# zhongyuanzhao/dl_ofdm

Measured on AMD Instinct MI355X. Metric: OFDM symbols/sec fwd+bwd, DCCN QPSK N=64, higher is better.
Workload: dtype f32; 1 GPU; QPSK, N=64/CP=16, batch=8192 OFDM symbols (1170 frames x 7), fwd+bwd+Adam; nfft=64, cp=16, nfilter=64, nbits=2, parallelism=independent batch per GPU, final all-reduce of the BER/loss table

## Files before the change

dl_ofdm_amd/csrc/dccn_abi.hip:

```cpp
#include "abi_impl.h"

namespace dccn {
thread_local int g_last_hip_error = 0;
thread_local ChainCtx tl_chain = {1, {{0, 0, 0, 0, 0, 0, 0, 0}}, {0, 0, 0, 0, 0, 0, 0, 0}, {0, 0, 0, 0, 0, 0, 0, 0}, {0, 0, 0, 0, 0, 0, 0, 0}, {0, 0, 0, 0, 0, 0, 0, 0}};
StepTraceState g_step_trace;
thread_local unsigned long long* tl_stamp = nullptr;

thread_local int tl_whole_k = -1;
thread_local int tl_tune_depth = 0;
thread_local int tl_tune_vals[TUNE_COUNT];
TuneTable g_tune = {{{9}, {7}, {7}, {7}, {0}, {0}, {0}, {1}, {1}, {1}, {1}, {1}, {3}, {1}, {14}, {0}, {0}, {1}, {0}, {2}, {1}, {1}, {0}, {0}, {1}, {2}, {0}, {1}}};
std::atomic<int> g_whole_k_global{1};

static int norm_grid_x(int cols) { return ceil_div(ceil_div(cols, 4), 64); }
static int norm_grid_y(int batch) { return ceil_div(batch, kNormRowsPerBlock); }

int norm_fused_blocks(int cols) { return ceil_div(ceil_div(cols, 4 * kNormFusedCG), 8) * 8; }
struct NormWs {
    double *moments, *power;
    size_t slots;
    double* power_slot(int slot) const { return power + (slot ? slots : 0); }
};
static NormWs norm_carve(Carver& c, int batch, int cols) {
    const size_t a = (size_t)norm_grid_x(cols) * norm_grid_y(batch), b = (size_t)norm_fused_blocks(cols), slots = a > b ? a : b;
// ... 651 lines not shown
    if (2 * kin == 160) DCCN_TRY(launch_rx_bwd_fused<5>(px, pw, de, nsplit, nr, fin, hp, s));
    else DCCN_TRY(launch_rx_bwd_fused<4>(px, pw, de, nsplit, nr, fin, hp, s));
    *ds = deferred_slabs(sw, dbias_dense != nullptr, true);
    fd->slabs = cw.partial; fd->colsum = cw.colsum;
    fd->splits = ceil_div(batch, 64) * S;
    fd->slab = (long long)((2 * F) / 64) * kin * 64;
    *fold_tilew = 64;
    return DCCN_OK;
}

static int tail_blocks(long long cells, bool quad4 = false) {
    long long b = ceil_div_ll(quad4 ? 4 * cells : cells, kTailThreads);
    const long long cap = quad4 ? kTailBlocksMax : kTailBlocks;
    if (b > cap) b = cap;
    if (b < 1) b = 1;
    return (int)b;
}
struct TailWs { TailBlockMetrics* blk_metrics; float* blk_grads; };
static TailWs tail_carve(Carver& c, size_t nblocks, int nbits) {
    TailBlockMetrics* bm = c.take<TailBlockMetrics>(nblocks);
    return TailWs{bm, c.take<float>(nblocks * tail_param_count(nbits))};
}
size_t tail_ws_bytes(long long cells, int nbits) {
    (void)cells;
    return carved_bytes([&](Carver& c) { tail_carve(c, kTailBlocksMax, nbits); });
}
static TailFinalizeArgs tail_finalize_args(const TailWs& w, int nblocks, bool bwd, int nbits, long long cells, dccn_metrics* metrics,
                                           float* dtailp, const PowerPartials* pp, float* power_out) {
    const bool pw = pp != nullptr && power_out != nullptr;
    TailFinalizeArgs fa{};
    fa.blk_metrics = w.blk_metrics; fa.blk_grads = bwd ? w.blk_grads : nullptr; fa.nblocks = nblocks;
    fa.P = bwd ? tail_param_count(nbits) : 0; fa.count = cells * nbits;
    fa.metrics = metrics; fa.dtailp = bwd ? dtailp : nullptr; fa.power_partial = pw ? pp->partial : nullptr;
    fa.n_power = pw ? pp->n : 0; fa.power_denom = pw ? pp->denom : 1.0; fa.power_out = pw ? power_out : nullptr;
    return fa;
}
static int tail_finish(const TailFinalizeArgs& fa, TailFinalizeArgs* defer, hipStream_t s) {
    if (defer) {
        *defer = fa;
        return DCCN_OK;
    }
    hipLaunchKernelGGL(demod_tail_finalize_kernel, dim3(tail_finalize_blocks(fa.P)), dim3(256), 0, s, fa);
    DCCN_LAUNCH_CHECK();
    return DCCN_OK;
}

template <int NB>
static int tail_launch(bool bwd, const float* z, const int32_t* bits, const float* tailp, float* prob, float* dz,
                       long long cells, int nblk, TailBlockMetrics* bm, float* bg, hipStream_t s) {
    if (bwd)
        DCCN_LAUNCH_CHAINS_Z((demod_tail_kernel<NB, true>), dim3(nblk), dim3(kTailThreads), 0, s, z, bits, tailp, prob,
                             dz, cells, bm, bg);
    else
        DCCN_LAUNCH_CHAINS_Z((demod_tail_kernel<NB, false>), dim3(nblk), dim3(kTailThreads), 0, s, z, bits, tailp, prob,
                             dz, cells, bm, bg);
    DCCN_LAUNCH_CHECK();
    return DCCN_OK;
}

int tail_impl(bool bwd, const float* z, const int32_t* bits, const float* tailp, float* prob,
                     dccn_metrics* metrics, float* dz, float* dtailp, long long cells, int nbits,
                     const PowerPartials* pp, float* power_out, void* ws, size_t ws_bytes, hipStream_t s,
                     TailFinalizeArgs* defer) {
    if (!z || !bits || !tailp || !metrics || cells <= 0 || nbits < 1 || nbits > 4) return DCCN_ERR_INVALID_ARG;
    if (bwd && (!dz || !dtailp)) return DCCN_ERR_INVALID_ARG;
    if (!ws || ws_bytes < tail_ws_bytes(cells, nbits)) return DCCN_ERR_WORKSPACE;
    Carver c(ws, ws_bytes);
    const TailWs tw = tail_carve(c, kTailBlocksMax, nbits);
    TailBlockMetrics* bm = tw.blk_metrics; float* bg = tw.blk_grads;
    const int nblk = tail_blocks(cells, bwd && nbits == 4);
    int st = DCCN_ERR_INVALID_ARG;
    switch (nbits) {
        case 1: st = tail_launch<1>(bwd, z, bits, tailp, prob, dz, cells, nblk, bm, bg, s); break;
        case 2: st = tail_launch<2>(bwd, z, bits, tailp, prob, dz, cells, nblk, bm, bg, s); break;
        case 3: st = tail_launch<3>(bwd, z, bits, tailp, prob, dz, cells, nblk, bm, bg, s); break;
        case 4:
            if (bwd) {
                if (prob)
                    DCCN_LAUNCH_CHAINS_Z(demod_tail_quad4_kernel<true>, dim3(nblk), dim3(kTailThreads), 0, s, z, bits, tailp,
                                         prob, dz, cells, bm, bg, tl_stamp);
                else
                    DCCN_LAUNCH_CHAINS_Z(demod_tail_quad4_kernel<false>, dim3(nblk), dim3(kTailThreads), 0, s, z, bits,
                                         tailp, prob, dz, cells, bm, bg, tl_stamp);
                DCCN_LAUNCH_CHECK();
                st = DCCN_OK;
            } else {
                st = tail_launch<4>(bwd, z, bits, tailp, prob, dz, cells, nblk, bm, bg, s);
            }
            break;
    }
    DCCN_TRY(st);
    if (!defer) DCCN_NO_CHAINS();
    return tail_finish(tail_finalize_args(tw, nblk, bwd, nbits, cells, metrics, dtailp, pp, power_out), defer, s);
}

static int dense_tail_max_blocks(int M, int N) {
    const int b = ceil_div(M, 32) * ceil_div(N, 64);
    const int few = (M <= 96 && (N % 16) == 0) ? ceil_div(M, 16) * (N / 16) : 0;
    return few > b && few <= kTailBlocksMax ? few : b;
}
size_t dense_tail_ws_bytes(int M, int N, int nbits) {
    return carved_bytes([&](Carver& c) { tail_carve(c, (size_t)dense_tail_max_blocks(M, N), nbits); });
}
static bool dense_tail_shape_ok(int M, int K, int N, int nbits) {
    return g_tune[TUNE_DENSE_FWD] > 0 && nbits >= 1 && nbits <= 4 && M > 0 && K > 0 && N > 0 && (K % 4 == 0) && (N % 4 == 0) &&
           small_enough(M, K) && small_enough(K, N) && (long long)ceil_div(M, 128) * ceil_div(N, 128) < 2 * kCUs;
}
bool dense_tail_ok(const float* x, const float* w, int M, int K, int N, int nbits) {
    return dense_tail_shape_ok(M, K, N, nbits) && aligned16(x) && aligned16(w);
}
bool dense_tail_planned(int nbits, bool train, int M, int N) {
    const int k = g_tune[TUNE_TAIL_FUSE_HI];
    if (nbits <= 2) return !((k & 4) && (long long)ceil_div(M, 128) * ceil_div(N, 128) >= 2 * kCUs);
    return (nbits == 4 && train) ? (k & 2) != 0 : (k & 1) != 0;
}

enum DenseGrid : int { DG_TILES = 0, DG_FEWROW, DG_RAGGED };
struct DenseRoute {
    DenseGrid grid;
    bool large;
    int rag;
    int blocks;
};
static DenseRoute dense_tail_route(const GemmParams& p, int nbits) {
    const int M = p.M, N = p.N, ncol = ceil_div(N, 64);
    DenseRoute r{};
    r.large = (long long)ceil_div(M, kDense48.rows()) * ncol >= 4LL * kCUs;
    constexpr int R = kDense80.rows();
    const int rag = (r.large && nbits <= 2 && g_tune[TUNE_DENSE_RAGGED] && M > R) ? M % R : 0;
    const int few_tiles = ceil_div(M, 16) * (N / 16);
    const bool few = g_tune[TUNE_FEWROW] && g_tune[TUNE_SKINNY] > 0 && nbits <= 2 && M <= 96 && fewrow_ng_c(p, false) >= 10 &&
                     few_tiles <= kTailBlocksMax && few_tiles <= dense_tail_max_blocks(M, N);
    if (rag > 0 && rag <= kDense32.rows()) {
        r.grid = DG_RAGGED; r.rag = rag; r.blocks = ((M - rag) / R) * ncol + ncol;
    } else if (few) {
        r.grid = DG_FEWROW; r.blocks = few_tiles;
    } else {
        r.grid = DG_TILES; r.blocks = ceil_div(M, r.large ? R : kDense48.rows()) * ncol;
    }
    return r;
}
static GemmParams split_last_rows(GemmParams& p, int rag) {
    GemmParams q = p;
    p.M -= rag;
    q.M = rag; q.A = p.A + (size_t)p.M * p.lda; q.C = p.C ? p.C + (size_t)p.M * p.ldc : nullptr;
    return q;
}

template <int NB, bool BWD>
static int dense_tail_launch(bool large, const GemmParams& p, const TailEpiParams& tp, hipStream_t s) {
    constexpr Tile16Cfg a = kDense48, b = kDense80;
    const size_t sm = tune_smem_min();
    if (large) return launch_dense_tail16<b.wgm, b.wgn, b.tm, b.tn, b.bk, b.ks, NB, BWD, 2>(p, tp, s, sm);
    return launch_dense_tail16<a.wgm, a.wgn, a.tm, a.tn, a.bk, a.ks, NB, BWD, 2>(p, tp, s, sm);
}

int dense_tail_impl(bool bwd, const float* x, const float* w, const float* bias, float* z, const int32_t* bits,
                           const float* tailp, float* prob, dccn_metrics* metrics, float* dz, float* dtailp, int M,
                           int K, int N, int nbits, const PowerPartials* pp, float* power_out, void* ws, size_t ws_bytes,
                           hipStream_t s, TailFinalizeArgs* defer) {
    if (!x || !w || !bits || !tailp || !metrics || M <= 0 || K <= 0 || N <= 0 || (N & 1) || nbits < 1 || nbits > 4)
        return DCCN_ERR_INVALID_ARG;
    if (bwd && (!dz || !dtailp)) return DCCN_ERR_INVALID_ARG;
    if (!dense_tail_ok(x, w, M, K, N, nbits)) return DCCN_ERR_INVALID_ARG;
    if (!ws || ws_bytes < dense_tail_ws_bytes(M, N, nbits)) return DCCN_ERR_WORKSPACE;
    const GemmParams p = dense_fwd_params(x, w, bias, z, M, K, N);
    if (!vec_both(p)) return DCCN_ERR_INVALID_ARG;
    const DenseRoute r = dense_tail_route(p, nbits);
    Carver c(ws, ws_bytes);
    const TailWs tw = tail_carve(c, (size_t)dense_tail_max_blocks(M, N), nbits);
    const long long cells = (long long)M * (N / 2);
    TailEpiParams tp;
    tp.bits = bits; tp.tailp = tailp; tp.prob = prob; tp.dz = dz; tp.blk_metrics = tw.blk_metrics; tp.blk_grads = tw.blk_grads;
    tp.inv_count = 1.0f / (float)(cells * nbits);
    int st;
    if (r.grid == DG_RAGGED) {
        GemmParams p1 = p;
        const GemmParams p2 = split_last_rows(p1, r.rag);
        const int M1 = p1.M;
        TailEpiParams t2 = tp;
        t2.bits = tp.bits + (size_t)M1 * (N / 2) * nbits;
        t2.prob = tp.prob ? tp.prob + (size_t)M1 * (N / 2) * nbits * 2 : nullptr;
        t2.dz = tp.dz ? tp.dz + (size_t)M1 * N : nullptr;
        constexpr Tile16Cfg c80 = kDense80, c32 = kDense32;
        const size_t sm = tune_smem_min();
        if (nbits == 1) st = bwd ? launch_dense_tail16_ragged<c80.tm, c32.tm, c80.bk, 1, true, 2>(p1, tp, p2, t2, s, sm) : launch_dense_tail16_ragged<c80.tm, c32.tm, c80.bk, 1, false, 2>(p1, tp, p2, t2, s, sm);
        else st = bwd ? launch_dense_tail16_ragged<c80.tm, c32.tm, c80.bk, 2, true, 2>(p1, tp, p2, t2, s, sm) : launch_dense_tail16_ragged<c80.tm, c32.tm, c80.bk, 2, false, 2>(p1, tp, p2, t2, s, sm);
    } else if (r.grid == DG_FEWROW) {
        if (nbits == 1) st = bwd ? launch_fewrow_tail<1, true>(p, tp, s) : launch_fewrow_tail<1, false>(p, tp, s);
        else st = bwd ? launch_fewrow_tail<2, true>(p, tp, s) : launch_fewrow_tail<2, false>(p, tp, s);
    }
    else if (nbits == 1) st = bwd ? dense_tail_launch<1, true>(r.large, p, tp, s) : dense_tail_launch<1, false>(r.large, p, tp, s);
    else if (nbits == 2) st = bwd ? dense_tail_launch<2, true>(r.large, p, tp, s) : dense_tail_launch<2, false>(r.large, p, tp, s);
    else if (nbits == 3) st = bwd ? dense_tail_launch<3, true>(r.large, p, tp, s) : dense_tail_launch<3, false>(r.large, p, tp, s);
    else st = bwd ? dense_tail_launch<4, true>(r.large, p, tp, s) : dense_tail_launch<4, false>(r.large, p, tp, s);
    DCCN_TRY(st);
    return tail_finish(tail_finalize_args(tw, r.blocks, bwd, nbits, cells, metrics, dtailp, pp, power_out), defer, s);
}

static int decide_row_bytes(int D, int nbits) { return (D * nbits + 7) / 8; }
bool decide_outputs_aligned(const float* llr, const float* prob, int nbits) {
    const uintptr_t la = nbits == 4 ? 15u : (nbits == 2 ? 7u : 3u);
    return (reinterpret_cast<uintptr_t>(llr) & la) == 0 && (reinterpret_cast<uintptr_t>(prob) & 7u) == 0;
}

int decide_impl(const float* z, const float* tailp, unsigned char* packed, float* llr, float* prob, int frames, int D,
                int nbits, hipStream_t s) {
    if (!z || !tailp || !packed || frames <= 0 || D <= 0 || nbits < 1 || nbits > 4) return DCCN_ERR_INVALID_ARG;
    if ((reinterpret_cast<uintptr_t>(z) & 7u) != 0 || !decide_outputs_aligned(llr, prob, nbits)) return DCCN_ERR_INVALID_ARG;
    const int gpr = ceil_div(D, 8), RB = decide_row_bytes(D, nbits);
    const long long blocks = ceil_div_ll((long long)frames * gpr * 8, kDecideThreads);
    if (blocks > 0x7fffffffLL) return DCCN_ERR_INVALID_ARG;
    const dim3 grid((unsigned)blocks), blk(kDecideThreads);
    switch (nbits) {
        case 1: DCCN_LAUNCH_CHAINS_Z(demod_decide_kernel<1>, grid, blk, 0, s, z, tailp, packed, llr, prob, frames, D, gpr, RB); break;
        case 2: DCCN_LAUNCH_CHAINS_Z(demod_decide_kernel<2>, grid, blk, 0, s, z, tailp, packed, llr, prob, frames, D, gpr, RB); break;
        case 3: DCCN_LAUNCH_CHAINS_Z(demod_decide_kernel<3>, grid, blk, 0, s, z, tailp, packed, llr, prob, frames, D, gpr, RB); break;
        default: DCCN_LAUNCH_CHAINS_Z(demod_decide_kernel<4>, grid, blk, 0, s, z, tailp, packed, llr, prob, frames, D, gpr, RB); break;
    }
    DCCN_LAUNCH_CHECK();
    return DCCN_OK;
}

int dense_decide_impl(const float* x, const float* w, const float* bias, float* z, const float* tailp, unsigned char* packed,
                      float* llr, float* prob, int M, int K, int N, int nbits, hipStream_t s) {
    if (!x || !w || !tailp || !packed || M <= 0 || K <= 0 || N <= 0 || (N & 1) || nbits < 1 || nbits > 4)
        return DCCN_ERR_INVALID_ARG;
    if (!dense_tail_ok(x, w, M, K, N, nbits)) return DCCN_ERR_INVALID_ARG;
    if (nbits >= 3 && !z) return DCCN_ERR_INVALID_ARG;
    if (!decide_outputs_aligned(llr, prob, nbits)) return DCCN_ERR_INVALID_ARG;
    const GemmParams p = dense_fwd_params(x, w, bias, z, M, K, N);
    if (!vec_both(p)) return DCCN_ERR_INVALID_ARG;
    const size_t sm = tune_smem_min();
    if (nbits >= 3) {
        DCCN_TRY(dense48_launch(p, s, sm));
        return decide_impl(z, tailp, packed, llr, prob, M, N / 2, nbits, s);
    }
    DecideEpiParams dq;
    dq.tailp = tailp; dq.packed = packed; dq.llr = llr; dq.prob = prob; dq.RB = decide_row_bytes(N / 2, nbits);
    const DenseRoute r = dense_tail_route(p, nbits);
    constexpr Tile16Cfg c48 = kDense48, c80 = kDense80, c32 = kDense32;
    if (r.grid == DG_RAGGED) {
        GemmParams p1 = p;
        const GemmParams p2 = split_last_rows(p1, r.rag);
        const int M1 = p1.M;
        DecideEpiParams d2 = dq;
        d2.packed = dq.packed + (size_t)M1 * dq.RB;
        d2.llr = dq.llr ? dq.llr + (size_t)M1 * (N / 2) * nbits : nullptr;
        d2.prob = dq.prob ? dq.prob + (size_t)M1 * (N / 2) * nbits * 2 : nullptr;
        return nbits == 1 ? launch_dense_decide16_ragged<c80.tm, c32.tm, c80.bk, 1, 2>(p1, dq, p2, d2, s, sm)
                          : launch_dense_decide16_ragged<c80.tm, c32.tm, c80.bk, 2, 2>(p1, dq, p2, d2, s, sm);
    }
    if (r.grid == DG_FEWROW) return nbits == 1 ? launch_fewrow_decide<1>(p, dq, s) : launch_fewrow_decide<2>(p, dq, s);
    if (r.large) return nbits == 1 ? launch_dense_decide16<c80.tm, c80.bk, 1, 2>(p, dq, s, sm) : launch_dense_decide16<c80.tm, c80.bk, 2, 2>(p, dq, s, sm);
    return nbits == 1 ? launch_dense_decide16<c48.tm, c48.bk, 1, 2>(p, dq, s, sm) : launch_dense_decide16<c48.tm, c48.bk, 2, 2>(p, dq, s, sm);
}

int adam_impl(float* param, const float* grad, float* m, float* v, const float* reg_coef,
                     const float* reg_gate, dccn_adam_state* st, dccn_adam_hparams hp, long long n, hipStream_t s,
                     bool prep) {
    if (!param || !grad || !m || !v || !st || n <= 0) return DCCN_ERR_INVALID_ARG;
    if (prep) {
        hipLaunchKernelGGL(adam_prep_kernel, dim3(1), dim3(64), 0, s, st, hp);
        DCCN_LAUNCH_CHECK();
    }
    long long blocks = ceil_div_ll(ceil_div_ll(n, 4), 256);
    if (blocks > 4 * kCUs) blocks = 4 * kCUs;
    hipLaunchKernelGGL(adam_apply_kernel, dim3((unsigned)blocks), dim3(256), 0, s, param, grad, m, v, reg_coef,
                       reg_gate, st, hp, n);
    DCCN_LAUNCH_CHECK();
    return DCCN_OK;
}

static bool shape_ok(const dccn_rx_shape* sh) {
    return sh && sh->batch > 0 && sh->S > 0 && sh->kin > 0 && sh->F > 0 && sh->D > 0 && sh->nbits >= 1 &&
           sh->nbits <= 4;
}

RxLayout rx_layout(const dccn_rx_shape* sh) {
    RxLayout L;
    const long long F2 = 2LL * sh->F;
    L.o_conv_w = 0;
    L.o_conv_b = L.o_conv_w + (long long)sh->kin * F2;
    L.o_dense_w = L.o_conv_b + F2;
    L.o_dense_b = L.o_dense_w + (long long)sh->S * F2 * 2 * sh->D;
    L.o_tail = L.o_dense_b + 2LL * sh->D;
    L.total = L.o_tail + tail_param_count(sh->nbits);
    L.rows = sh->batch * sh->S;
    L.cols = sh->S * sh->kin * 2;
    L.dK = sh->S * sh->F * 2;
    L.dN = 2 * sh->D;
    L.cells = (long long)sh->batch * sh->D;
    L.ws_norm = norm_ws_bytes(sh->batch, L.cols);
    L.ws_tail = tail_ws_bytes(L.cells, sh->nbits);
    {
        const size_t f = dense_tail_ws_bytes(sh->batch, L.dN, sh->nbits);
        if (f > L.ws_tail) L.ws_tail = f;
    }
    L.ws_dense_bw = splitk_ws_bytes(L.dK, L.dN, sh->batch);
    L.ws_conv_bw = cconv_bw_ws_bytes(L.rows, sh->kin, sh->F);
    {
        const size_t f = rx_bwd_fused_ws_bytes(sh->batch, sh->S, sh->kin, sh->F);
        if (2LL * sh->kin <= 192 && f > L.ws_conv_bw) L.ws_conv_bw = f;
    }
    return L;
}
enum RxMode : int { RX_RECEIVE = 0, RX_EVAL, RX_TRAIN };
struct RxWs { void *norm, *tail, *dense_bw, *conv_bw; };
static RxWs rx_carve(Carver& c, const RxLayout& L, RxMode mode) {
    RxWs w{};
    w.norm = c.take<char>(L.ws_norm);
    if (mode >= RX_EVAL) w.tail = c.take<char>(L.ws_tail);
    if (mode == RX_TRAIN) {
        w.dense_bw = c.take<char>(L.ws_dense_bw);
        w.conv_bw = c.take<char>(L.ws_conv_bw);
    }
    return w;
}
static size_t rx_ws_bytes(const dccn_rx_shape* sh, RxMode mode) {
    const RxLayout L = rx_layout(sh);
    return carved_bytes([&](Carver& c) { rx_carve(c, L, mode); });
}

struct OverlapStreams {
    hipStream_t side;
    hipEvent_t fork, join;
};
static bool overlap_streams(OverlapStreams* o) {
    static std::mutex mu;
    static hipStream_t sides[64];
    thread_local hipEvent_t ev[64][2];
    int dev = 0;
    if (hipGetDevice(&dev) != hipSuccess || dev < 0 || dev >= 64) return false;
    {
        std::lock_guard<std::mutex> lock(mu);
        if (!sides[dev]) {
            int least = 0, greatest = 0;
            if (hipDeviceGetStreamPriorityRange(&least, &greatest) != hipSuccess) least = 0;
            if (hipStreamCreateWithPriority(&sides[dev], hipStreamNonBlocking, least) != hipSuccess) { sides[dev] = nullptr; return false; }
        }
    }
    for (int k = 0; k < 2; ++k)
        if (!ev[dev][k] && hipEventCreateWithFlags(&ev[dev][k], hipEventDisableTiming) != hipSuccess) { ev[dev][k] = nullptr; return false; }
    o->side = sides[dev]; o->fork = ev[dev][0]; o->join = ev[dev][1];
    return true;
}

bool gen_static_doppler(const dccn_gen_static* g) {
    if (!g || g->doppler_period <= 0) return false;
    if (g->n_profiles == 0) return !g->identity && g->Fd > 0.1f;
    for (int i = 0; i < g->n_profiles; ++i)
        if (!g->profiles[i].identity && g->profiles[i].Fd > 0.1f) return true;
    return false;
}
bool gen_static_shape_ok(int S, int K, int CP) { return S == 7 && K == 64 && (CP == 16 || CP == 4); }
static_assert(gen_static_smem_bytes<7, 64, 4>() == 18112, "short prefix: 16 x 132 grid floats + 2 x (476 + 128) samples");
bool gen_static_ok(const dccn_gen_static* g) {
    if (!g || !g->bits_out || !g->cell_map || !g->const_tab || !g->idft || !g->snr_db || !g->y || !g->noise || !g->power_partial)
        return false;
    if (g->frames <= 0 || g->frames > 65535 || g->S <= 0 || 2 * g->S > 16 || g->K <= 0 || g->CP < 0 || g->D <= 0 || g->nbits < 1 ||
        g->nbits > 4 || (g->n_profiles == 0 && (g->L <= 0 || g->L > 64)))
        return false;
    if (g->n_profiles < 0 || g->n_profiles > kGenMaxProfiles || (g->n_profiles > 0 && !g->profiles) || g->tap_stride < 0 ||
        (g->H_out && g->h_rep <= 0))
        return false;
    if (g->n_profiles == 0) {
        if (!g->identity && (!g->coeff || !g->alpha || g->n_taps <= 0 || g->n_taps > 16)) return false;
        if (g->tap_stride != 0 && g->tap_stride < g->n_taps) return false;
    }
    for (int i = 0; i < g->n_profiles; ++i) {
        const dccn_gen_profile& q = g->profiles[i];
        if (q.L <= 0 || q.L > 64) return false;
        if (!q.identity && (!q.coeff || !q.alpha || q.n_taps <= 0 || q.n_taps > 16 || g->tap_stride < q.n_taps)) return false;
    }
    if (g->doppler_period < 0) return false;
    if (g->doppler_period > 0) {
        if (!(g->t_sym > 0.f) || !std::isfinite(g->t_sym)) return false;
        if (g->n_profiles == 0 && !std::isfinite(g->Fd)) return false;
        for (int i = 0; i < g->n_profiles; ++i)
            if (!std::isfinite(g->profiles[i].Fd)) return false;
        if (gen_static_doppler(g) && g->H_out && g->h_rep != g->S) return false;
    }
    return gen_static_shape_ok(g->S, g->K, g->CP) && aligned16(g->y) && aligned16(g->noise);
}
int gen_static_args(const dccn_gen_static* g, GenStaticArgs* out) {
    if (!gen_static_ok(g)) return DCCN_ERR_INVALID_ARG;
    if (ceil_div(g->frames, kGenFramesPerBlock) > kChanPartials) return DCCN_ERR_INVALID_ARG;
    GenStaticArgs& a = *out;
    a.bits_out = g->bits_out; a.cell_map = g->cell_map; a.const_tab = reinterpret_cast<const float2*>(g->const_tab);
    a.pilot = make_float2(g->pilot_re, g->pilot_im); a.idft = g->idft;
    memset(a.prof, 0, sizeof(a.prof));
    if (g->n_profiles == 0) {
        a.prof[0].coeff = g->coeff; a.prof[0].alpha = g->alpha; a.prof[0].n_taps = g->n_taps; a.prof[0].L = g->L;
        a.prof[0].identity = g->identity; a.prof[0].Fd = g->Fd;
        a.n_prof = 1;
        a.tap_stride = g->tap_stride > 0 ? g->tap_stride : g->n_taps;
    } else {
        for (int i = 0; i < g->n_profiles; ++i) {
            a.prof[i].coeff = g->profiles[i].coeff; a.prof[i].alpha = g->profiles[i].alpha;
            a.prof[i].n_taps = g->profiles[i].n_taps; a.prof[i].L = g->profiles[i].L; a.prof[i].identity = g->profiles[i].identity;
            a.prof[i].Fd = g->profiles[i].Fd;
        }
        a.n_prof = g->n_profiles;
        a.tap_stride = g->tap_stride;
    }
    a.H = reinterpret_cast<float2*>(g->H_out); a.h_rep = g->h_rep;
    a.dop_period = gen_static_doppler(g) ? g->doppler_period : 0; a.t_sym = g->t_sym;
    a.snr_db = g->snr_db; a.y = reinterpret_cast<float2*>(g->y); a.noise = reinterpret_cast<float2*>(g->noise);
// ... 801 lines not shown
```

dl_ofdm_amd/csrc/gemm16.h:

```cpp
#pragma once
#include <algorithm>
#include "gemm_f32_mfma.h"
#include "tail.h"
#include "decide.h"

#ifndef GEMM16_ABL
#define GEMM16_ABL 0
#endif

namespace dccn {

typedef float f32x4 __attribute__((ext_vector_type(4)));

enum Epilogue16 : int { EPI_STORE = 0, EPI_TAIL = 1, EPI_DECIDE = 2 };

struct TailEpiParams {
    const int32_t* bits;
    const float* tailp;
    float* prob;
    float* dz;
    TailBlockMetrics* blk_metrics;
    float* blk_grads;
    float inv_count;
    __device__ __forceinline__ TailEpiParams at_chain(const long long off) const {
        TailEpiParams q = *this;
        q.bits = chain_at(bits, off); q.tailp = chain_at(tailp, off); q.prob = chain_at(prob, off); q.dz = chain_at(dz, off);
        q.blk_metrics = chain_at(blk_metrics, off); q.blk_grads = chain_at(blk_grads, off);
        return q;
    }
};

template <int KIND, int BI, int BK, int NT>
struct Tile16 {
    static_assert(BK % 32 == 0 && BI % 16 == 0, "tile shape");
    static_assert(KIND == OP_ICONTIG || KIND == OP_KCONTIG || KIND == OP_CCONV_W, "operand kind");
    static constexpr int K4 = BK / 4;
    static constexpr int LD = BK + 8;
    static constexpr bool IC = (KIND == OP_ICONTIG);
    static constexpr bool CC = (KIND == OP_CCONV_W);
    static constexpr int UNITS = IC ? (BI / 4) * K4 : BI * K4;
    static constexpr int NU = (UNITS + NT - 1) / NT;
    static constexpr int NV = IC ? 4 * NU : NU;
    static constexpr int NOFF = CC ? 2 * NV : NV;
    float4 r[2][NV];
    unsigned voff[NOFF];
    unsigned soff[NU];
    unsigned okmask;

    static __device__ __forceinline__ int unit_index(int u, int tid) { return (tid + u * NT) % UNITS; }
    static __device__ __forceinline__ void ic_coords(int bidx, int& i4, int& k4) {
        const int sub = bidx & 7, rest = bidx >> 3;
        i4 = rest % (BI / 4);
        k4 = (rest / (BI / 4)) * 8 + sub;
    }

    __device__ __forceinline__ void init(int ld, int i0, int I, int cF, int tid) {
        okmask = 0u;
#pragma unroll
        for (int u = 0; u < NU; ++u) {
            const int idx = unit_index(u, tid);
            if constexpr (IC) {
                int i4, k4;
                ic_coords(idx, i4, k4);
                soff[u] = (unsigned)((4 * i4) * LD + 4 * k4);
#pragma unroll
                for (int e = 0; e < 4; ++e)
                    voff[4 * u + e] = (unsigned)(((4 * k4 + e) * ld + min(i0 + 4 * i4, I - 4)) * 4);
            } else {
                soff[u] = (unsigned)((idx / K4) * LD + (idx % K4) * 4);
                const int ic = min(i0 + idx / K4, I - 1);
                const int k = (idx % K4) * 4;
                if constexpr (KIND == OP_KCONTIG) {
                    voff[u] = (unsigned)((ic * ld + k) * 4);
                } else {
                    const int f = ic >> 1, c = ic & 1, n0 = k >> 1;
                    voff[2 * u] = (unsigned)((n0 * 2 * cF + f + (c ? cF : 0)) * 4);
                    voff[2 * u + 1] = (unsigned)((n0 * 2 * cF + f + (c ? 0 : cF)) * 4);
                }
            }
        }
    }
    static __device__ __forceinline__ const char* tile_base(const float* p, int ld, int k0, int cF) {
        if constexpr (KIND == OP_ICONTIG) return reinterpret_cast<const char*>(p + (size_t)k0 * ld);
        else if constexpr (KIND == OP_KCONTIG) return reinterpret_cast<const char*>(p + k0);
        else return reinterpret_cast<const char*>(p + (size_t)(k0 >> 1) * 2 * cF);
    }
    __device__ __forceinline__ void load_fast(int v, const char* __restrict__ base, int cF, int s = 0) {
        if constexpr (!CC) {
            r[s][v] = *reinterpret_cast<const float4*>(base + voff[v]);
        } else {
            const unsigned row = (unsigned)(2 * cF * 4);
            const float a0 = *reinterpret_cast<const float*>(base + voff[2 * v]);
            const float b0 = *reinterpret_cast<const float*>(base + voff[2 * v + 1]);
            const float a1 = *reinterpret_cast<const float*>(base + voff[2 * v] + row);
            const float b1 = *reinterpret_cast<const float*>(base + voff[2 * v + 1] + row);
            r[s][v] = make_float4(a0, -b0, a1, -b1);
        }
    }

    __device__ __forceinline__ void load_masked(int v, const float* __restrict__ p, int ld, int k0, int kend, int K,
                                                int i0, int I, int cF, int tid) {
        const int u = IC ? v / 4 : v;
        const int idx = unit_index(u, tid);
        if constexpr (IC) {
            int i4, k4;
            ic_coords(idx, i4, k4);
            const int k = k0 + 4 * k4 + (v & 3);
            r[0][v] = *reinterpret_cast<const float4*>(p + (size_t)min(k, K - 1) * ld + min(i0 + 4 * i4, I - 4));
            okmask = (okmask & ~(1u << v)) | ((k < kend ? 1u : 0u) << v);
        } else {
            const int ic = min(i0 + idx / K4, I - 1);
            const int k = k0 + (idx % K4) * 4;
            const int kc = min(k, K - 4);
            if constexpr (KIND == OP_KCONTIG) {
                r[0][v] = *reinterpret_cast<const float4*>(p + (size_t)ic * ld + kc);
            } else {
                r[0][v] = make_float4(cconv_weff(p, cF, kc, ic), cconv_weff(p, cF, kc + 1, ic), cconv_weff(p, cF, kc + 2, ic),
                                   cconv_weff(p, cF, kc + 3, ic));
            }
            okmask = (okmask & ~(1u << v)) | ((k < kend ? 1u : 0u) << v);
        }
    }

    template <bool MASKED>
    __device__ __forceinline__ void store_piece(int v, float* __restrict__ lds, int s = 0) const {
        if constexpr (IC) {
            const int b = v & ~3, q = v & 3;
            float4 val = make_float4(f4c(r[s][b + 0], q), f4c(r[s][b + 1], q), f4c(r[s][b + 2], q), f4c(r[s][b + 3], q));
            if constexpr (MASKED) {
                val.x = ((okmask >> (b + 0)) & 1u) ? val.x : 0.f;
                val.y = ((okmask >> (b + 1)) & 1u) ? val.y : 0.f;
                val.z = ((okmask >> (b + 2)) & 1u) ? val.z : 0.f;
                val.w = ((okmask >> (b + 3)) & 1u) ? val.w : 0.f;
            }
            *reinterpret_cast<float4*>(lds + soff[v / 4] + q * LD) = val;
        } else {
            float4 val = r[s][v];
            if constexpr (MASKED) {
                const bool ok = (okmask >> v) & 1u;
                val = make_float4(ok ? val.x : 0.f, ok ? val.y : 0.f, ok ? val.z : 0.f, ok ? val.w : 0.f);
            }
            *reinterpret_cast<float4*>(lds + soff[v]) = val;
        }
    }
};

template <int KA, int KB, int WGM, int WGN, int TM, int TN, int BK, int KS>
struct Cfg16 {
    static constexpr int NT = 256 * KS;
    static constexpr int BM = WGM * TM * 16, BN = WGN * TN * 16;
    using TA = Tile16<KA, BM, BK, NT>;
    using TB = Tile16<KB, BN, BK, NT>;
    static constexpr size_t tile_bytes = (size_t)(2 * BM * TA::LD + 2 * BN * TB::LD) * sizeof(float);
    static constexpr size_t xchg_bytes = KS > 1 ? (size_t)KS * 4 * TM * TN * 4 * 64 * sizeof(float) : 0;
    static constexpr size_t smem_bytes(int tail_floats) {
        const size_t e = xchg_bytes + (size_t)tail_floats * sizeof(float) + 16;
        return tile_bytes > e ? tile_bytes : e;
    }
};

template <class CF, int NB, bool BWD>
struct TailLds16 {
    static constexpr bool STAGED = NB >= 3;
    static constexpr bool QUAD4 = NB == 4 && BWD;
    static_assert(!STAGED || CF::xchg_bytes == 0, "LDS-staged tail: one wave set");
    static constexpr int ZS = CF::BN + 2;
    static constexpr int TCELLS = CF::BM * (CF::BN / 2);
    static constexpr int PW = tail_param_count(NB);
    static constexpr int zt = 0;
    static constexpr int lt = CF::BM * ZS;
    static constexpr int swl = lt + TCELLS;
    static constexpr int red = STAGED ? swl + ((PW + 3) & ~3) : (int)(CF::xchg_bytes / sizeof(float));
    static constexpr int red_floats = QUAD4 ? tail_quad4_lds_floats(CF::NT) : tail_reduce_lds_floats<NB, BWD>(CF::NT);
    static constexpr size_t bytes = CF::smem_bytes((STAGED ? red : 0) + red_floats);
};

template <int W, bool DZ>
struct TailOutTile {
    float* pb[W];
    float* db[W];
    unsigned lp, ld;
    __device__ __forceinline__ bool any_prob() const { return pb[0] != nullptr; }
    __device__ __forceinline__ void prob(const int u, const int j, const float p0, const float p1) const {
        *reinterpret_cast<float2*>(pb[u] + lp + 2 * j) = make_float2(p0, p1);
    }
    __device__ __forceinline__ void dz(const int u, const float d0, const float d1) const {
        if constexpr (DZ) out_store2<1>(db[u] + ld, d0, d1);
    }
};

constexpr int tail_batch_width(const int ncell) {
    return ncell <= 8 ? ncell : (ncell % 8 == 0 ? 8 : (ncell % 6 == 0 ? 6 : (ncell % 5 == 0 ? 5 : 4)));
}

template <int KA, int KB, int WGM, int WGN, int TM, int TN, int BK, int KS, int COLSUM, int EPI, int NB, bool BWD,
          int PD = 1>
__device__ __forceinline__ void gemm16_block(const GemmParams& p, const TailEpiParams& tp, const int L, const int T,
                                             const int z, const int slab, const DecideEpiParams* dp = nullptr) {
    static_assert(WGM * WGN == 4, "four waves per wave set");
    using CF = Cfg16<KA, KB, WGM, WGN, TM, TN, BK, KS>;
    using TA = typename CF::TA;
    using TB = typename CF::TB;
    constexpr int NT = CF::NT, BM = CF::BM, BN = CF::BN;
    constexpr int LDA = TA::LD, LDB = TB::LD;
    extern __shared__ __attribute__((aligned(16))) float smem[];
    float* sA = smem;
    float* sB = smem + 2 * BM * LDA;

    const int tid = threadIdx.x;
    const int lane = tid & 63, wid = (tid >> 6) & 3, set = tid >> 8;
    const int l15 = lane & 15, kg = lane >> 4;
    const int wm0 = (wid / WGN) * (TM * 16), wn0 = (wid % WGN) * (TN * 16);
    const int ntn = (p.N + BN - 1) / BN;
    int tile;
    {
        const int xcd = L & 7, j = L >> 3, q = T >> 3, r = T & 7;
        tile = (xcd < r ? xcd * (q + 1) : r * (q + 1) + (xcd - r) * q) + j;
    }
    const int m0 = (tile / ntn) * BM, n0 = (tile % ntn) * BN;
    const int kbeg = z * p.klen;
    const int kend = min(p.K, kbeg + p.klen);
    const int ntiles = (kend - kbeg + BK - 1) / BK;
    const int nfull = (kend - kbeg) / BK;

    f32x4 acc[TM][TN];
#pragma unroll
    for (int a = 0; a < TM; ++a)
#pragma unroll
        for (int b = 0; b < TN; ++b)
#pragma unroll
            for (int r = 0; r < 4; ++r) acc[a][b][r] = 0.f;

    float cs = 0.f;
    const bool do_cs = COLSUM && p.colsum != nullptr && m0 == 0 && tid < BN;

    static_assert(EPI == EPI_STORE || (NB >= 1 && NB <= 4), "EPI_TAIL / EPI_DECIDE: NB is bits per symbol");
    constexpr int NCELL = (EPI == EPI_TAIL) ? TM * TN * 2 / KS : 1;
    constexpr bool TAIL_LDS = (EPI == EPI_TAIL) && NB >= 3;
    constexpr bool QUAD4 = TAIL_LDS && NB == 4 && BWD;
    static_assert(!TAIL_LDS || KS == 1, "LDS-staged tail: one wave set");
    constexpr int TCELLS = BM * (BN / 2);
    constexpr int CPT = TAIL_LDS ? (TCELLS + NT - 1) / NT : 1;
    int plab[CPT];
    if constexpr (TAIL_LDS) {
#pragma unroll
        for (int i = 0; i < CPT; ++i) {
            const int c = min(tid + NT * i, TCELLS - 1);
            const int row = min(m0 + c / (BN / 2), p.M - 1), dc = min((n0 >> 1) + c % (BN / 2), (p.N >> 1) - 1);
            const int32_t* lb = tp.bits + ((long long)row * (p.N >> 1) + dc) * NB;
            int v = 0;
#pragma unroll
            for (int j = 0; j < NB; ++j) v |= (lb[j] != 0 ? 1 : 0) << j;
            plab[i] = v;
        }
    }
    int labs[NCELL][NB];
    if constexpr (EPI == EPI_TAIL && !TAIL_LDS) {
#pragma unroll
        for (int a = 0; a < TM; ++a)
#pragma unroll
            for (int b = 0; b < TN; ++b)
#pragma unroll
                for (int cc = 0; cc < 2 / KS; ++cc) {
                    const int c = KS > 1 ? set : cc;
                    const int row = min(m0 + wm0 + a * 16 + 4 * kg + ((lane & 1) ? 2 + c : c), p.M - 1);
                    const int col = min(n0 + wn0 + b * 16 + l15, p.N - 1);
                    const long long cell = (long long)row * (p.N >> 1) + (col >> 1);
#pragma unroll
                    for (int j = 0; j < NB; ++j) labs[(a * TN + b) * (2 / KS) + cc][j] = tp.bits[cell * NB + j];
                }
    }

    float bjv[(EPI != EPI_STORE) ? TN : 1];
    if constexpr (EPI != EPI_STORE) {
#pragma unroll
        for (int b = 0; b < TN; ++b) bjv[b] = p.bias != nullptr ? p.bias[min(n0 + wn0 + b * 16 + l15, p.N - 1)] : 0.f;
    }

    TA ta;
    TB tb;
    ta.init(p.lda, m0, p.M, p.cF, tid);
    tb.init(p.ldb, n0, p.N, p.cF, tid);
    constexpr int PA = TA::NV, PB = TB::NV;
    constexpr int NG = BK / 16;
    static_assert(NG % KS == 0, "k-tile groups must split evenly over the wave sets");
    constexpr int NGS = NG / KS;
    constexpr int NSTEP = NGS * 4;
    constexpr int HALF = NSTEP / 2;
    constexpr int LPS = (PA + PB + HALF - 1) / HALF;

    using I0 = std::integral_constant<int, 0>;
    using I1 = std::integral_constant<int, 1>;
    using I2 = std::integral_constant<int, 2>;
    auto load_ab = [&](auto mode_tag, auto set_tag, int q, int k0) {
        constexpr int MODE = decltype(mode_tag)::value, RS = decltype(set_tag)::value;
        if (q < PA) {
            if constexpr (MODE == PF_FAST) ta.load_fast(q, TA::tile_base(p.A, p.lda, k0, p.cF), p.cF, RS);
            else ta.load_masked(q, p.A, p.lda, k0, kend, p.K, m0, p.M, p.cF, tid);
        } else {
            if constexpr (MODE == PF_FAST) tb.load_fast(q - PA, TB::tile_base(p.B, p.ldb, k0, p.cF), p.cF, RS);
            else tb.load_masked(q - PA, p.B, p.ldb, k0, kend, p.K, n0, p.N, p.cF, tid);
        }
    };
    auto store_ab = [&](auto mode_tag, int q, float* An, float* Bn) {
        constexpr int MODE = decltype(mode_tag)::value;
        if (q < PA) ta.template store_piece<MODE == PF_MASKED>(q, An);
        else tb.template store_piece<MODE == PF_MASKED>(q - PA, Bn);
    };
    auto stage_first = [&](auto mode_tag) {
#pragma unroll
        for (int q = 0; q < PA + PB; ++q) load_ab(mode_tag, I0{}, q, kbeg);
#pragma unroll
        for (int q = 0; q < PA + PB; ++q) store_ab(mode_tag, q, sA, sB);
    };
    if (ntiles > 0) {
        if (nfull > 0) stage_first(std::integral_constant<int, PF_FAST>{});
        else stage_first(std::integral_constant<int, PF_MASKED>{});
    }
    __syncthreads();

    int t = 0;
    auto ktile2 = [&](auto load_tag, auto store_tag, auto lset_tag, auto sset_tag, auto dist_tag) {
        constexpr int LMODE = decltype(load_tag)::value, SMODE = decltype(store_tag)::value;
        constexpr int SSET = decltype(sset_tag)::value, DIST = decltype(dist_tag)::value;
        const int cur = t & 1;
        const int k0n = kbeg + (t + DIST) * BK;
        const float* As = sA + cur * BM * LDA + (wm0 + l15) * LDA + 4 * kg + 16 * NGS * set;
        const float* Bs = sB + cur * BN * LDB + (wn0 + l15) * LDB + 4 * kg + 16 * NGS * set;
        float* An = sA + (cur ^ 1) * BM * LDA;
        float* Bn = sB + (cur ^ 1) * BN * LDB;
        float4 fa[2][TM], fb[2][TN];
#pragma unroll
        for (int a = 0; a < TM; ++a) fa[0][a] = *reinterpret_cast<const float4*>(As + a * 16 * LDA);
#pragma unroll
        for (int b = 0; b < TN; ++b) fb[0][b] = *reinterpret_cast<const float4*>(Bs + b * 16 * LDB);
#pragma unroll
        for (int g = 0; g < NGS; ++g) {
            if (g + 1 < NGS && !(GEMM16_ABL & 8)) {
#pragma unroll
                for (int a = 0; a < TM; ++a)
                    fa[(g + 1) & 1][a] = *reinterpret_cast<const float4*>(As + a * 16 * LDA + 16 * (g + 1));
#pragma unroll
                for (int b = 0; b < TN; ++b)
                    fb[(g + 1) & 1][b] = *reinterpret_cast<const float4*>(Bs + b * 16 * LDB + 16 * (g + 1));
            }
#pragma unroll
            for (int j = 0; j < 4; ++j) {
                const int step = g * 4 + j;
                if constexpr (LMODE != PF_NONE && !(GEMM16_ABL & 1)) {
                    if (step < HALF) {
#pragma unroll
                        for (int q = step * LPS; q < (step + 1) * LPS && q < PA + PB; ++q) load_ab(load_tag, lset_tag, q, k0n);
                    }
                }
                __builtin_amdgcn_sched_barrier(0);
#pragma unroll
                for (int a = 0; a < TM; ++a)
#pragma unroll
                    for (int b = 0; b < TN; ++b)
                        acc[a][b] = __builtin_amdgcn_mfma_f32_16x16x4f32(f4c(fa[g & 1][a], j), f4c(fb[g & 1][b], j),
                                                                         acc[a][b], 0, 0, 0);
                __builtin_amdgcn_sched_barrier(0);
                if constexpr (SMODE != PF_NONE && !(GEMM16_ABL & 2)) {
                    if (step >= HALF) {
#pragma unroll
                        for (int q = (step - HALF) * LPS; q < (step - HALF + 1) * LPS && q < PA + PB; ++q) {
                            if (q < PA) ta.template store_piece<SMODE == PF_MASKED>(q, An, SSET);
                            else tb.template store_piece<SMODE == PF_MASKED>(q - PA, Bn, SSET);
                        }
                    }
                }
            }
        }
        if (COLSUM && do_cs) {
            const float* Bc = sB + cur * BN * LDB + tid * LDB;
#pragma unroll
            for (int k = 0; k < BK; k += 4) {
                const float4 v = *reinterpret_cast<const float4*>(Bc + k);
                cs += (v.x + v.y) + (v.z + v.w);
            }
        }
        if constexpr (!(GEMM16_ABL & 4)) __syncthreads();
        ++t;
    };
    using TF = std::integral_constant<int, PF_FAST>;
    using TM_ = std::integral_constant<int, PF_MASKED>;
    using TN_ = std::integral_constant<int, PF_NONE>;
    bool deep = false;
    if constexpr (PD == 2) deep = nfull == ntiles && ntiles >= 2;
    if (deep) {
#pragma unroll
        for (int q = 0; q < PA + PB; ++q) load_ab(TF{}, I1{}, q, kbeg + BK);
        while (t + 3 < ntiles) {
            ktile2(TF{}, TF{}, I0{}, I1{}, I2{});
            ktile2(TF{}, TF{}, I1{}, I0{}, I2{});
        }
        const int rem = ntiles - t;
        if (rem == 3) {
            ktile2(TF{}, TF{}, I0{}, I1{}, I2{});
            ktile2(TN_{}, TF{}, I1{}, I0{}, I2{});
            ktile2(TN_{}, TN_{}, I0{}, I0{}, I2{});
        } else if (rem == 2) {
            ktile2(TN_{}, TF{}, I0{}, I1{}, I2{});
            ktile2(TN_{}, TN_{}, I0{}, I0{}, I2{});
        } else {
            ktile2(TN_{}, TN_{}, I0{}, I0{}, I2{});
        }
    } else {
        while (t + 1 < nfull) ktile2(TF{}, TF{}, I0{}, I0{}, I1{});
        while (t + 1 < ntiles) ktile2(TM_{}, TM_{}, I0{}, I0{}, I1{});
        if (ntiles > 0) ktile2(TN_{}, TN_{}, I0{}, I0{}, I1{});
    }

    if (COLSUM && do_cs) {
        const int col = n0 + tid;
        if (col < p.N) p.colsum[(size_t)z * p.N + col] = cs;
    }

    float* xch = smem;
    if constexpr (KS > 1) {
#pragma unroll
        for (int a = 0; a < TM; ++a)
#pragma unroll
            for (int b = 0; b < TN; ++b)
#pragma unroll
                for (int r = 0; r < 4; ++r)
                    xch[(((set * 4 + wid) * (TM * TN) + a * TN + b) * 4 + r) * 64 + lane] = acc[a][b][r];
        __syncthreads();
    }
    auto tile_val = [&](int a, int b, int r, int ln) -> float {
        if constexpr (KS > 1) {
            float v = xch[(((0 * 4 + wid) * (TM * TN) + a * TN + b) * 4 + r) * 64 + ln];
#pragma unroll
            for (int s2 = 1; s2 < KS; ++s2) v += xch[(((s2 * 4 + wid) * (TM * TN) + a * TN + b) * 4 + r) * 64 + ln];
            return v;
        } else {
            return acc[a][b][r];
        }
    };
    static_assert(KS == 1 || KS == 2, "wave sets");

    if constexpr (EPI == EPI_STORE) {
        constexpr int STAGE = NB;
        static_assert(STAGE >= STORE_PLAIN && STAGE <= STORE_EQUALISE, "EPI_STORE: a StoreStage");
        float* Cz = p.C + (size_t)z * p.slab;
#pragma unroll
        for (int a = 0; a < TM; ++a) {
#pragma unroll
            for (int b = 0; b < TN; ++b) {
                const int col = n0 + wn0 + b * 16 + l15;
                float bj = 0.f;
                if (p.bias != nullptr && col < p.N) {
                    if (p.cbias) {
                        const float d = p.bias[col >> 1] - p.bias[p.cF + (col >> 1)];
                        bj = (col & 1) ? -d : d;
                    } else {
                        bj = p.bias[col];
                    }
                }
#pragma unroll
                for (int rr = 0; rr < 4 / KS; ++rr) {
                    const int r = KS > 1 ? 2 * set + rr : rr;
                    const int row = m0 + wm0 + a * 16 + 4 * kg + r;
                    float v;
                    if constexpr (KS > 1) v = set == 0 ? tile_val(a, b, rr, lane) : tile_val(a, b, 2 + rr, lane);
                    else v = acc[a][b][rr];
                    if constexpr (STAGE == STORE_EQUALISE) {
                        static_assert(KS == 1, "equalise stage: one wave set");
                        const float o = v + bj;
                        const float partner = __shfl_xor(o, 1, 64);
                        if (row < p.M && col < p.N) {
                            const size_t ci = (size_t)row * p.ldc + col, c0 = ci - (size_t)(col & 1);
                            Cz[ci] = o;
                            const float hr = (col & 1) ? partner : o, hi = (col & 1) ? o : partner;
                            const float2 yv = *reinterpret_cast<const float2*>(p.aux + c0);
                            const float aa = sqrtf(hr * hr + hi * hi);
                            const float cr = hr / aa, cim = (-hi) / aa;
                            const float er = yv.x * cr - yv.y * cim, ei = yv.x * cim + yv.y * cr;
                            if ((col & 1) == 0) *reinterpret_cast<float2*>(p.out2 + c0) = make_float2(er, ei);
                            else *reinterpret_cast<float2*>(p.out3 + c0) = make_float2(er * er - ei * (-ei), er * (-ei) + ei * er);
                        }
                    } else
                    if (row < p.M && col < p.N) {
                        const size_t ci = (size_t)row * p.ldc + col;
                        float auxv = 0.f;
                        if constexpr (store_stage_reads_aux(STAGE)) auxv = p.aux[ci];
                        Cz[ci] = store_stage<STAGE>(v + bj, auxv);
                    }
                }
            }
        }
    } else if constexpr (EPI == EPI_DECIDE) {
        static_assert(KS == 1 && NB <= 2 && WGM == 1 && WGN == 4 && TN == 1, "decision epilogue: 16 TM x 64 tiles, BPSK / QPSK");
        const DecideEpiParams& dq = *dp;
        const int odd = lane & 1;
        const int Dn = p.N >> 1;
        constexpr int NC = TM * 2;
        float cz0[NC], cz1[NC];
        bool cvalid[NC];
        float* cprob[NC];
        float* cllr[NC];
        int crl[NC];
#pragma unroll
        for (int a = 0; a < TM; ++a) {
            const int col = n0 + wn0 + l15;
            const int colc = min(col, p.N - 1);
            const float bj = bjv[0];
            const float o0 = acc[a][0][0] + bj, o1 = acc[a][0][1] + bj, o2 = acc[a][0][2] + bj, o3 = acc[a][0][3] + bj;
            const float t0 = __builtin_bit_cast(float, dpp_mov_i32(__builtin_bit_cast(int, o0), 0));
            const float t1 = __builtin_bit_cast(float, dpp_mov_i32(__builtin_bit_cast(int, o1), 0));
            const float t2 = __builtin_bit_cast(float, dpp_mov_i32(__builtin_bit_cast(int, o2), 0));
            const float t3 = __builtin_bit_cast(float, dpp_mov_i32(__builtin_bit_cast(int, o3), 0));
            if (p.C != nullptr) {
                const int row = m0 + wm0 + a * 16 + 4 * kg;
                if (col < p.N) {
                    if (row + 0 < p.M) p.C[(size_t)(row + 0) * p.ldc + col] = o0;
                    if (row + 1 < p.M) p.C[(size_t)(row + 1) * p.ldc + col] = o1;
                    if (row + 2 < p.M) p.C[(size_t)(row + 2) * p.ldc + col] = o2;
                    if (row + 3 < p.M) p.C[(size_t)(row + 3) * p.ldc + col] = o3;
                }
            }
            const float mine0 = odd ? o2 : o0, mine1 = odd ? o3 : o1;
            const float othr0 = odd ? t2 : t0, othr1 = odd ? t3 : t1;
#pragma unroll
            for (int cc = 0; cc < 2; ++cc) {
                const int ci = a * 2 + cc;
                const float mine = cc ? mine1 : mine0, othr = cc ? othr1 : othr0;
                cz0[ci] = odd ? othr : mine;
                cz1[ci] = odd ? mine : othr;
                const int rl = wm0 + a * 16 + 4 * kg + (odd ? 2 : 0) + cc;
                const int row = m0 + rl;
                const bool ok = row < p.M && col < p.N;
                const long long cell = (long long)min(row, p.M - 1) * Dn + (colc >> 1);
                crl[ci] = rl;
                cvalid[ci] = ok;
                cprob[ci] = (dq.prob != nullptr && ok) ? dq.prob + cell * NB * 2 : nullptr;
                cllr[ci] = (dq.llr != nullptr && ok) ? dq.llr + cell * NB : nullptr;
            }
        }
        unsigned hard[NC];
        {
            constexpr int TW = tail_batch_width(NC);
            static_assert(NC % TW == 0, "decision batches");
#pragma unroll
            for (int g0 = 0; g0 < NC; g0 += TW) {
                float a0[TW], a1[TW];
                float* pc[TW];
                float* lc[TW];
                unsigned hd[TW];
#pragma unroll
                for (int u = 0; u < TW; ++u) { a0[u] = cz0[g0 + u]; a1[u] = cz1[g0 + u]; pc[u] = cprob[g0 + u]; lc[u] = cllr[g0 + u]; }
                decide_cells<NB, TW>(a0, a1, dq.tailp, pc, lc, hd);
#pragma unroll
                for (int u = 0; u < TW; ++u) hard[g0 + u] = hd[u];
            }
        }
        unsigned short* sb = reinterpret_cast<unsigned short*>(smem);
#pragma unroll
        for (int ci = 0; ci < NC; ++ci) {
// ... 389 lines not shown
```

Measured before the change: 117.7 million OFDM symbols/s.

## Add PD=3 deep K-loop pipeline with early shared-memory stores for small dense GEMMs

Adds a third pipeline depth mode to the 16x16 MFMA GEMM. It prefetches two K tiles into registers, writes the next tile to the LDS double buffer during the first half of the MFMA steps, and reads the next tile's first fragment group before the loop boundary, so each K tile needs only one barrier. An empty asm constraint pins the prefetched registers so the compiler cannot move the loads next to their use. The kDense48 tail and decide launches now use this depth; the cost is higher register pressure and stricter shape requirements (even group count, no column sums).

Result: no change. 118.2 million OFDM symbols/s, median of 6 (+0.4%).

```diff
diff --git a/dl_ofdm_amd/csrc/dccn_abi.hip b/dl_ofdm_amd/csrc/dccn_abi.hip
--- a/dl_ofdm_amd/csrc/dccn_abi.hip
+++ b/dl_ofdm_amd/csrc/dccn_abi.hip
@@ -827,7 +827,7 @@
     constexpr Tile16Cfg a = kDense48, b = kDense80;
     const size_t sm = tune_smem_min();
     if (large) return launch_dense_tail16<b.wgm, b.wgn, b.tm, b.tn, b.bk, b.ks, NB, BWD, 2>(p, tp, s, sm);
-    return launch_dense_tail16<a.wgm, a.wgn, a.tm, a.tn, a.bk, a.ks, NB, BWD, 2>(p, tp, s, sm);
+    return launch_dense_tail16<a.wgm, a.wgn, a.tm, a.tn, a.bk, a.ks, NB, BWD, 3>(p, tp, s, sm);
 }
 
 int dense_tail_impl(bool bwd, const float* x, const float* w, const float* bias, float* z, const int32_t* bits,
@@ -928,7 +928,7 @@
     }
     if (r.grid == DG_FEWROW) return nbits == 1 ? launch_fewrow_decide<1>(p, dq, s) : launch_fewrow_decide<2>(p, dq, s);
     if (r.large) return nbits == 1 ? launch_dense_decide16<c80.tm, c80.bk, 1, 2>(p, dq, s, sm) : launch_dense_decide16<c80.tm, c80.bk, 2, 2>(p, dq, s, sm);
-    return nbits == 1 ? launch_dense_decide16<c48.tm, c48.bk, 1, 2>(p, dq, s, sm) : launch_dense_decide16<c48.tm, c48.bk, 2, 2>(p, dq, s, sm);
+    return nbits == 1 ? launch_dense_decide16<c48.tm, c48.bk, 1, 3>(p, dq, s, sm) : launch_dense_decide16<c48.tm, c48.bk, 2, 3>(p, dq, s, sm);
 }
 
 int adam_impl(float* param, const float* grad, float* m, float* v, const float* reg_coef,
diff --git a/dl_ofdm_amd/csrc/gemm16.h b/dl_ofdm_amd/csrc/gemm16.h
--- a/dl_ofdm_amd/csrc/gemm16.h
+++ b/dl_ofdm_amd/csrc/gemm16.h
@@ -122,10 +122,19 @@
         }
     }
 
-    template <bool MASKED>
-    __device__ __forceinline__ void store_piece(int v, float* __restrict__ lds, int s = 0) const {
+    template <bool MASKED, bool PIN = false>
+    __device__ __forceinline__ void store_piece(int v, float* __restrict__ lds, int s = 0) {
         if constexpr (IC) {
             const int b = v & ~3, q = v & 3;
+            if constexpr (PIN) {
+                if (q == 0) {
+                    f32x4 t0 = __builtin_bit_cast(f32x4, r[s][b + 0]), t1 = __builtin_bit_cast(f32x4, r[s][b + 1]);
+                    f32x4 t2 = __builtin_bit_cast(f32x4, r[s][b + 2]), t3 = __builtin_bit_cast(f32x4, r[s][b + 3]);
+                    asm volatile("" : "+v"(t0), "+v"(t1), "+v"(t2), "+v"(t3));
+                    r[s][b + 0] = __builtin_bit_cast(float4, t0); r[s][b + 1] = __builtin_bit_cast(float4, t1);
+                    r[s][b + 2] = __builtin_bit_cast(float4, t2); r[s][b + 3] = __builtin_bit_cast(float4, t3);
+                }
+            }
             float4 val = make_float4(f4c(r[s][b + 0], q), f4c(r[s][b + 1], q), f4c(r[s][b + 2], q), f4c(r[s][b + 3], q));
             if constexpr (MASKED) {
                 val.x = ((okmask >> (b + 0)) & 1u) ? val.x : 0.f;
@@ -291,7 +300,6 @@
 
     using I0 = std::integral_constant<int, 0>;
     using I1 = std::integral_constant<int, 1>;
-    using I2 = std::integral_constant<int, 2>;
     auto load_ab = [&](auto mode_tag, auto set_tag, int q, int k0) {
         constexpr int MODE = decltype(mode_tag)::value, RS = decltype(set_tag)::value;
         if (q < PA) {
@@ -302,20 +310,31 @@
             else tb.load_masked(q - PA, p.B, p.ldb, k0, kend, p.K, n0, p.N, p.cF, tid);
         }
     };
-    auto store_ab = [&](auto mode_tag, int q, float* An, float* Bn) {
+    auto store_ab = [&](auto mode_tag, auto pin_tag, int q, float* An, float* Bn) {
         constexpr int MODE = decltype(mode_tag)::value;
-        if (q < PA) ta.template store_piece<MODE == PF_MASKED>(q, An);
-        else tb.template store_piece<MODE == PF_MASKED>(q - PA, Bn);
+        constexpr bool PIN = decltype(pin_tag)::value;
+        if (q < PA) ta.template store_piece<MODE == PF_MASKED, PIN>(q, An);
+        else tb.template store_piece<MODE == PF_MASKED, PIN>(q - PA, Bn);
     };
-    auto stage_first = [&](auto mode_tag) {
+    constexpr bool DEEP_OK = PD >= 2;
+    static_assert(PD == 1 || PD == 2 || (PD == 3 && !COLSUM && NGS % 2 == 0), "PD = 3: even group count, no column sums");
+    bool deep = false;
+    if constexpr (DEEP_OK) deep = nfull == ntiles && ntiles >= 2;
+    auto stage_first = [&](auto mode_tag, auto deep_tag) {
 #pragma unroll
         for (int q = 0; q < PA + PB; ++q) load_ab(mode_tag, I0{}, q, kbeg);
-#pragma unroll
-        for (int q = 0; q < PA + PB; ++q) store_ab(mode_tag, q, sA, sB);
+        if constexpr (decltype(deep_tag)::value) {
+#pragma unroll
+            for (int q = 0; q < PA + PB; ++q) load_ab(mode_tag, I1{}, q, kbeg + BK);
+        }
+#pragma unroll
+        for (int q = 0; q < PA + PB; ++q) store_ab(mode_tag, deep_tag, q, sA, sB);
     };
-    if (ntiles > 0) {
-        if (nfull > 0) stage_first(std::integral_constant<int, PF_FAST>{});
-        else stage_first(std::integral_constant<int, PF_MASKED>{});
+    if (deep) {
+        stage_first(std::integral_constant<int, PF_FAST>{}, std::true_type{});
+    } else if (ntiles > 0) {
+        if (nfull > 0) stage_first(std::integral_constant<int, PF_FAST>{}, std::false_type{});
+        else stage_first(std::integral_constant<int, PF_MASKED>{}, std::false_type{});
     }
     __syncthreads();
 
@@ -365,8 +384,8 @@
                     if (step >= HALF) {
 #pragma unroll
                         for (int q = (step - HALF) * LPS; q < (step - HALF + 1) * LPS && q < PA + PB; ++q) {
-                            if (q < PA) ta.template store_piece<SMODE == PF_MASKED>(q, An, SSET);
-                            else tb.template store_piece<SMODE == PF_MASKED>(q - PA, Bn, SSET);
+                            if (q < PA) ta.template store_piece<SMODE == PF_MASKED, DIST == 2>(q, An, SSET);
+                            else tb.template store_piece<SMODE == PF_MASKED, DIST == 2>(q - PA, Bn, SSET);
                         }
                     }
                 }
@@ -386,25 +405,99 @@
     using TF = std::integral_constant<int, PF_FAST>;
     using TM_ = std::integral_constant<int, PF_MASKED>;
     using TN_ = std::integral_constant<int, PF_NONE>;
-    bool deep = false;
-    if constexpr (PD == 2) deep = nfull == ntiles && ntiles >= 2;
+    float4 dfa[2][TM], dfb[2][TN];
+    auto read_group = [&](const int buf, const int g, const int slot) {
+        const float* As = sA + buf * BM * LDA + (wm0 + l15) * LDA + 4 * kg + 16 * NGS * set + 16 * g;
+        const float* Bs = sB + buf * BN * LDB + (wn0 + l15) * LDB + 4 * kg + 16 * NGS * set + 16 * g;
+#pragma unroll
+        for (int a = 0; a < TM; ++a) dfa[slot][a] = *reinterpret_cast<const float4*>(As + a * 16 * LDA);
+#pragma unroll
+        for (int b = 0; b < TN; ++b) dfb[slot][b] = *reinterpret_cast<const float4*>(Bs + b * 16 * LDB);
+    };
+    auto ktile_deep = [&](auto load_tag, auto next_tag, auto lset_tag, auto sset_tag) {
+        constexpr bool LOAD = decltype(load_tag)::value;
+        constexpr bool NEXT = decltype(next_tag)::value;
+        constexpr int SSET = decltype(sset_tag)::value;
+        const int cur = t & 1;
+        const int k0n = kbeg + (t + 2) * BK;
+        float* An = sA + (cur ^ 1) * BM * LDA;
+        float* Bn = sB + (cur ^ 1) * BN * LDB;
+#pragma unroll
+        for (int g = 0; g < NGS; ++g) {
+            if (g + 1 == NGS) {
+                if constexpr (!(GEMM16_ABL & 4)) __syncthreads();
+                if constexpr (NEXT && !(GEMM16_ABL & 8)) read_group(cur ^ 1, 0, 0);
+            }
+#pragma unroll
+            for (int j = 0; j < 4; ++j) {
+                const int step = g * 4 + j;
+                if constexpr (!(GEMM16_ABL & 8)) {
+                    if (g + 1 < NGS && j == (g == 0 ? 1 : 0)) read_group(cur, g + 1, (g + 1) & 1);
+                }
+                if constexpr (LOAD && !(GEMM16_ABL & 1)) {
+                    if (step < HALF) {
+#pragma unroll
+                        for (int q = step * LPS; q < (step + 1) * LPS && q < PA + PB; ++q) load_ab(TF{}, lset_tag, q, k0n);
+                    }
+                }
+                __builtin_amdgcn_sched_barrier(0);
+#pragma unroll
+                for (int a = 0; a < TM; ++a)
+#pragma unroll
+                    for (int b = 0; b < TN; ++b)
+                        acc[a][b] = __builtin_amdgcn_mfma_f32_16x16x4f32(f4c(dfa[g & 1][a], j), f4c(dfb[g & 1][b], j),
+                                                                         acc[a][b], 0, 0, 0);
+                __builtin_amdgcn_sched_barrier(0);
+                if constexpr (NEXT && !(GEMM16_ABL & 2)) {
+                    if (step < HALF) {
+#pragma unroll
+                        for (int q = step * LPS; q < (step + 1) * LPS && q < PA + PB; ++q) {
+                            if (q < PA) ta.template store_piece<false, true>(q, An, SSET);
+                            else tb.template store_piece<false, true>(q - PA, Bn, SSET);
+                        }
+                    }
+                }
+            }
+        }
+        ++t;
+    };
+    using Y = std::true_type;
+    using N = std::false_type;
+    using I2 = std::integral_constant<int, 2>;
     if (deep) {
-#pragma unroll
-        for (int q = 0; q < PA + PB; ++q) load_ab(TF{}, I1{}, q, kbeg + BK);
-        while (t + 3 < ntiles) {
-            ktile2(TF{}, TF{}, I0{}, I1{}, I2{});
-            ktile2(TF{}, TF{}, I1{}, I0{}, I2{});
-        }
-        const int rem = ntiles - t;
-        if (rem == 3) {
-            ktile2(TF{}, TF{}, I0{}, I1{}, I2{});
-            ktile2(TN_{}, TF{}, I1{}, I0{}, I2{});
-            ktile2(TN_{}, TN_{}, I0{}, I0{}, I2{});
-        } else if (rem == 2) {
-            ktile2(TN_{}, TF{}, I0{}, I1{}, I2{});
-            ktile2(TN_{}, TN_{}, I0{}, I0{}, I2{});
-        } else {
-            ktile2(TN_{}, TN_{}, I0{}, I0{}, I2{});
+        if constexpr (PD == 2) {
+            while (t + 3 < ntiles) {
+                ktile2(TF{}, TF{}, I0{}, I1{}, I2{});
+                ktile2(TF{}, TF{}, I1{}, I0{}, I2{});
+            }
+            const int rem = ntiles - t;
+            if (rem == 3) {
+                ktile2(TF{}, TF{}, I0{}, I1{}, I2{});
+                ktile2(TN_{}, TF{}, I1{}, I0{}, I2{});
+                ktile2(TN_{}, TN_{}, I0{}, I0{}, I2{});
+            } else if (rem == 2) {
+                ktile2(TN_{}, TF{}, I0{}, I1{}, I2{});
+                ktile2(TN_{}, TN_{}, I0{}, I0{}, I2{});
+            } else {
+                ktile2(TN_{}, TN_{}, I0{}, I0{}, I2{});
+            }
+        } else if constexpr (PD == 3) {
+            read_group(0, 0, 0);
+            while (t + 3 < ntiles) {
+                ktile_deep(Y{}, Y{}, I0{}, I1{});
+                ktile_deep(Y{}, Y{}, I1{}, I0{});
+            }
+            const int rem = ntiles - t;
+            if (rem == 3) {
+                ktile_deep(Y{}, Y{}, I0{}, I1{});
+                ktile_deep(N{}, Y{}, I1{}, I0{});
+                ktile_deep(N{}, N{}, I0{}, I0{});
+            } else if (rem == 2) {
+                ktile_deep(N{}, Y{}, I0{}, I1{});
+                ktile_deep(N{}, N{}, I0{}, I0{});
+            } else {
+                ktile_deep(N{}, N{}, I0{}, I0{});
+            }
         }
     } else {
         while (t + 1 < nfull) ktile2(TF{}, TF{}, I0{}, I0{}, I1{});
```
